# qzs634/Probabilistic-Multiplanar-Unet

Hardware: AMD Instinct MI355X
Metric: 2D slices/sec fwd+bwd, 256×256×1 batch32 U-Net; Dice vs ref (higher is better)
Workload: dtype fp32; 1 GPU; c2: UNet(n_channels=1, n_classes=1, num_filters=[64, 128, 256, 512, 1024]), 256x256x1 slices, fwd+BCE+bwd+clip(0.1)+SGD(0.9) per step, fp32; global_batch=32, per_gpu_batch=32, parallelism=dp1

## Files before the change

### probabilistic-multiplanar-unet_amd/csrc/conv3x3_wino4.hip

```cpp
#include <string.h>
#include <stdlib.h>
#include <utility>
#include "pmu_common.h"
#include "pmu_lds.h"

namespace {

constexpr int TX = 8, TY = 8;
constexpr int OW = 4 * TX, OH = 4 * TY;
constexpr int HW = OW + 2, HH = OH + 2;
constexpr int BK = 8;
constexpr int GP = 36;
constexpr int ROWF = 312;
constexpr int ROWU = ROWF / 4;
constexpr int A_FLOATS = HH * ROWF;
constexpr int CO = 32;
constexpr int NC = 36;
constexpr int U_FLOATS = BK * CO * NC;
constexpr int STAGE = A_FLOATS + U_FLOATS;
constexpr int NT = 512;
constexpr int A_UNITS = A_FLOATS / 4;
constexpr int NGL = (A_UNITS + NT - 1) / NT;
constexpr int UGL = (U_FLOATS / 4 + NT - 1) / NT;
constexpr int RED_FLOATS = 8 * 16 * 2;
static_assert(U_FLOATS % (4 * 256) == 0, "U of whole wave DMA instructions");
static_assert((2 * STAGE + RED_FLOATS) * 4 <= 160 * 1024, "LDS");

struct W4Args {
  const float* x;
  const float* wp;
  const float* bias;
  float* out0;
  float* out1;
  float* part;
  int H, W, KC, NOUT, split, bw, bh, nco, cpb;
  int prio;
  int ts, tc;
  int N;
  const float* bz;
  const float* bcoef;
  const float* bmean;
  const float* binv;
};

constexpr int upos(int ch, int cl) { return cl < 16 ? 16 * ch + cl : 32 + 2 * ch + (cl - 16); }

__device__ __forceinline__ void g6(const double (&g)[3], double (&t)[6]) {
  t[0] = g[0] / 4.0;
  t[1] = -(g[0] + g[1] + g[2]) / 6.0;
  t[2] = -(g[0] - g[1] + g[2]) / 6.0;
  t[3] = g[0] / 24.0 + g[1] / 12.0 + g[2] / 6.0;
  t[4] = g[0] / 24.0 - g[1] / 12.0 + g[2] / 6.0;
  t[5] = g[2];
}

__device__ __forceinline__ void pack_wino4_body(const float* __restrict__ w, int Cout, int Cin, int dgrad,
                                                float* __restrict__ wp, int bid) {
  constexpr int SEG = BK * CO * NC;
  __shared__ float4 seg4[SEG / 4];
  const int NOUT = dgrad ? Cin : Cout, KC = dgrad ? Cout : Cin;
  const int nch = (KC + BK - 1) / BK;
  const int ch = bid % nch, jb = bid / nch;
  for (int f = threadIdx.x; f < BK * CO; f += blockDim.x) {
    const int col = dgrad ? f % CO : f / BK, kl = dgrad ? f / CO : f % BK;
    const int j = jb * CO + col, k = ch * BK + kl;
    double g[3][3];
    for (int a = 0; a < 3; ++a)
      for (int b = 0; b < 3; ++b) {
        double v = 0.0;
        if (j < NOUT && k < KC)
          v = dgrad ? w[((long long)k * Cin + j) * 9 + (2 - a) * 3 + (2 - b)] : w[((long long)j * Cin + k) * 9 + a * 3 + b];
        g[a][b] = v;
      }
    double t[6][3];
    for (int b = 0; b < 3; ++b) {
      const double col3[3] = {g[0][b], g[1][b], g[2][b]};
      double o[6];
      g6(col3, o);
      for (int a = 0; a < 6; ++a) t[a][b] = o[a];
    }
    float u[36];
    for (int a = 0; a < 6; ++a) {
      const double row3[3] = {t[a][0], t[a][1], t[a][2]};
      double o[6];
      g6(row3, o);
      for (int b = 0; b < 6; ++b) u[6 * a + b] = (float)o[b];
    }
    float row[36];
    for (int c = 0; c < 36; ++c) row[upos(c / 18, c % 18)] = u[c];
    float4* d = seg4 + (kl * CO + col) * (NC / 4);
    for (int q = 0; q < 9; ++q) d[q] = make_float4(row[4 * q], row[4 * q + 1], row[4 * q + 2], row[4 * q + 3]);
  }
  __syncthreads();
  float4* dst = reinterpret_cast<float4*>(wp + (long long)bid * SEG);
  for (int i = threadIdx.x; i < SEG / 4; i += blockDim.x) dst[i] = seg4[i];
}
__global__ __launch_bounds__(256) void pack_wino4_kernel(const float* __restrict__ w, int Cout, int Cin, int dgrad,
                                                         float* __restrict__ wp) {
  pack_wino4_body(w, Cout, Cin, dgrad, wp, blockIdx.x);
}
__global__ __launch_bounds__(256) void pack_wino4_multi_kernel(const pmu_pack_job* __restrict__ jobs, int njobs,
                                                               int dgrad) {
  const pmu_pack_job& j = jobs[pmu_job_of(jobs, njobs, blockIdx.x)];
  pack_wino4_body(j.w, j.Cout, j.Cin, dgrad, (float*)j.dst, blockIdx.x - j.block0);
}

__device__ __forceinline__ void bt6(float d0, float d1, float d2, float d3, float d4, float d5, float& r0, float& r1,
                                    float& r2, float& r3, float& r4, float& r5) {
  r0 = fmaf(-5.f, d2, fmaf(4.f, d0, d4));
  const float a = fmaf(-4.f, d2, d4), b = fmaf(-4.f, d1, d3);
  r1 = a + b;
  r2 = a - b;
  const float c = d4 - d2, e = d3 - d1;
  r3 = fmaf(2.f, e, c);
  r4 = fmaf(-2.f, e, c);
  r5 = fmaf(-5.f, d3, fmaf(4.f, d1, d5));
}

__device__ __forceinline__ void input_transform4(const float (&d)[36], float (&v)[36]) {
  float t[36];
#pragma unroll
  for (int j = 0; j < 6; ++j)
    bt6(d[j], d[6 + j], d[12 + j], d[18 + j], d[24 + j], d[30 + j], t[j], t[6 + j], t[12 + j], t[18 + j], t[24 + j],
        t[30 + j]);
#pragma unroll
  for (int a = 0; a < 6; ++a)
    bt6(t[6 * a], t[6 * a + 1], t[6 * a + 2], t[6 * a + 3], t[6 * a + 4], t[6 * a + 5], v[6 * a], v[6 * a + 1],
        v[6 * a + 2], v[6 * a + 3], v[6 * a + 4], v[6 * a + 5]);
}

__device__ __forceinline__ void at4(float m0, float m1, float m2, float m3, float m4, float m5, float& y0, float& y1,
                                    float& y2, float& y3) {
  const float s12 = m1 + m2, d12 = m1 - m2, s34 = m3 + m4, d34 = m3 - m4;
  y0 = m0 + s12 + s34;
  y1 = fmaf(2.f, d34, d12);
  y2 = fmaf(4.f, s34, s12);
  y3 = fmaf(8.f, d34, d12) + m5;
}

template <int E>
struct PatchOff {
  static constexpr int value = ((E / 6) * ROWF + ((E % 6) >> 2) * GP + ((E % 6) & 3) * 8) * 4;
};
template <int E0, int N>
__device__ __forceinline__ void load_patch_part(unsigned pa, float (&d)[36]) {
  if constexpr (N > 0) {
    d[E0] = lds_b32<PatchOff<E0>::value>(pa);
    load_patch_part<E0 + 1, N - 1>(pa, d);
  }
}

template <int CH>
__device__ __forceinline__ void input_transform_half(const float (&d)[36], float (&v)[18]) {
  float t[18];
#pragma unroll
  for (int j = 0; j < 6; ++j) {
    const float d0 = d[j], d1 = d[6 + j], d2 = d[12 + j], d3 = d[18 + j], d4 = d[24 + j], d5 = d[30 + j];
    if (CH == 0) {
      t[j] = fmaf(-5.f, d2, fmaf(4.f, d0, d4));
      const float a = fmaf(-4.f, d2, d4), b = fmaf(-4.f, d1, d3);
      t[6 + j] = a + b;
      t[12 + j] = a - b;
    } else {
      const float c = d4 - d2, e = d3 - d1;
      t[j] = fmaf(2.f, e, c);
      t[6 + j] = fmaf(-2.f, e, c);
      t[12 + j] = fmaf(-5.f, d3, fmaf(4.f, d1, d5));
    }
  }
#pragma unroll
  for (int a = 0; a < 3; ++a)
    bt6(t[6 * a], t[6 * a + 1], t[6 * a + 2], t[6 * a + 3], t[6 * a + 4], t[6 * a + 5], v[6 * a], v[6 * a + 1],
        v[6 * a + 2], v[6 * a + 3], v[6 * a + 4], v[6 * a + 5]);
}

template <int CH, int G>
__device__ __forceinline__ void w4_uread(unsigned ua, float4 (&ur)[3][2], float2 (&ut)[2]) {
  if constexpr (G < 4) {
    ur[G % 3][0] = lds_b128<upos(CH, 4 * G) * 4>(ua);
    ur[G % 3][1] = lds_b128<(16 * NC + upos(CH, 4 * G)) * 4>(ua);
  } else {
    ut[0] = lds_b64<upos(CH, 16) * 4>(ua);
    ut[1] = lds_b64<(16 * NC + upos(CH, 16)) * 4>(ua);
  }
}

template <int CH, int G, bool PF>
__device__ __forceinline__ void w4_group(unsigned ua, const float (&v)[18], float4 (&ur)[3][2], float2 (&ut)[2],
                                         f32x4 (&acc)[2][18], unsigned pn, float (&dn)[36]) {
  if constexpr (G > 0) wait_lgkm<(PF && G == 4) ? 12 : 2 * ((G + 2 < 4 ? G + 2 : 4) - G)>();
  __builtin_amdgcn_sched_barrier(0);
  if constexpr (G < 4) {
    constexpr int c0 = 4 * G;
#pragma unroll
    for (int h = 0; h < 2; ++h) {
      const float4 q = ur[G % 3][h];
      acc[h][c0 + 0] = mfma16(v[c0 + 0], q.x, acc[h][c0 + 0]);
      acc[h][c0 + 1] = mfma16(v[c0 + 1], q.y, acc[h][c0 + 1]);
      acc[h][c0 + 2] = mfma16(v[c0 + 2], q.z, acc[h][c0 + 2]);
      acc[h][c0 + 3] = mfma16(v[c0 + 3], q.w, acc[h][c0 + 3]);
    }
  } else {
#pragma unroll
    for (int h = 0; h < 2; ++h) {
      acc[h][16] = mfma16(v[16], ut[h].x, acc[h][16]);
      acc[h][17] = mfma16(v[17], ut[h].y, acc[h][17]);
    }
  }
  __builtin_amdgcn_sched_barrier(0);
  if constexpr (G + 3 <= 4) w4_uread<CH, G + 3>(ua, ur, ut);
  if constexpr (PF && G == 3) load_patch_part<0, 12>(pn, dn);
  if constexpr (PF && G == 4) load_patch_part<12, 24>(pn, dn);
}

template <int CH, bool PF>
__device__ __forceinline__ void w4_chunk(unsigned pa, unsigned ua, f32x4 (&acc)[2][18]) {
  float d[36], v[18];
  float4 ur[3][2];
  float2 ut[2];
  load_patch_part<0, 36>(pa, d);
  w4_uread<CH, 0>(ua, ur, ut);
  w4_uread<CH, 1>(ua, ur, ut);
  w4_uread<CH, 2>(ua, ur, ut);
  wait_lgkm<4>();
  __builtin_amdgcn_sched_barrier(0);
  input_transform_half<CH>(d, v);
  __builtin_amdgcn_sched_barrier(0);
  const unsigned pa1 = pa + 4, ua1 = ua + CO * NC * 4;
  w4_group<CH, 0, PF>(ua, v, ur, ut, acc, pa1, d);
  w4_group<CH, 1, PF>(ua, v, ur, ut, acc, pa1, d);
  w4_group<CH, 2, PF>(ua, v, ur, ut, acc, pa1, d);
  w4_group<CH, 3, PF>(ua, v, ur, ut, acc, pa1, d);
  w4_group<CH, 4, PF>(ua, v, ur, ut, acc, pa1, d);
  if constexpr (!PF) load_patch_part<0, 36>(pa1, d);
  w4_uread<CH, 0>(ua1, ur, ut);
  w4_uread<CH, 1>(ua1, ur, ut);
  w4_uread<CH, 2>(ua1, ur, ut);
  wait_lgkm<4>();
  __builtin_amdgcn_sched_barrier(0);
  input_transform_half<CH>(d, v);
  __builtin_amdgcn_sched_barrier(0);
  w4_group<CH, 0, false>(ua1, v, ur, ut, acc, pa1, d);
  w4_group<CH, 1, false>(ua1, v, ur, ut, acc, pa1, d);
  w4_group<CH, 2, false>(ua1, v, ur, ut, acc, pa1, d);
  w4_group<CH, 3, false>(ua1, v, ur, ut, acc, pa1, d);
  w4_group<CH, 4, false>(ua1, v, ur, ut, acc, pa1, d);
}

template <int CH>
__device__ __forceinline__ void w4_col_half(float d0, float d1, float d2, float d3, float d4, float d5, float& r0,
                                            float& r1, float& r2) {
  if (CH == 0) {
    r0 = fmaf(-5.f, d2, fmaf(4.f, d0, d4));
    const float a = fmaf(-4.f, d2, d4), b = fmaf(-4.f, d1, d3);
    r1 = a + b;
    r2 = a - b;
  } else {
    const float c = d4 - d2, e = d3 - d1;
    r0 = fmaf(2.f, e, c);
    r1 = fmaf(-2.f, e, c);
    r2 = fmaf(-5.f, d3, fmaf(4.f, d1, d5));
  }
}
template <int CH, int J>
__device__ __forceinline__ void w4_col_read(unsigned pa, float2 (&c)[5]) {
  c[0] = lds_b64<PatchOff<6 * CH + J>::value>(pa);
  c[1] = lds_b64<PatchOff<6 * CH + 6 + J>::value>(pa);
  c[2] = lds_b64<PatchOff<6 * CH + 12 + J>::value>(pa);
  c[3] = lds_b64<PatchOff<6 * CH + 18 + J>::value>(pa);
  c[4] = lds_b64<PatchOff<6 * CH + 24 + J>::value>(pa);
}
template <int CH, int J>
__device__ __forceinline__ void w4_col_tf(const float2 (&c)[5], float (&t0)[18], float (&t1)[18]) {
  if (CH == 0) {
    w4_col_half<0>(c[0].x, c[1].x, c[2].x, c[3].x, c[4].x, 0.f, t0[J], t0[6 + J], t0[12 + J]);
    w4_col_half<0>(c[0].y, c[1].y, c[2].y, c[3].y, c[4].y, 0.f, t1[J], t1[6 + J], t1[12 + J]);
  } else {
    w4_col_half<1>(0.f, c[0].x, c[1].x, c[2].x, c[3].x, c[4].x, t0[J], t0[6 + J], t0[12 + J]);
    w4_col_half<1>(0.f, c[0].y, c[1].y, c[2].y, c[3].y, c[4].y, t1[J], t1[6 + J], t1[12 + J]);
  }
}
template <int CH>
__device__ __forceinline__ void w4_row_pass(const float (&t)[18], float (&v)[18]) {
#pragma unroll
  for (int a = 0; a < 3; ++a)
    bt6(t[6 * a], t[6 * a + 1], t[6 * a + 2], t[6 * a + 3], t[6 * a + 4], t[6 * a + 5], v[6 * a], v[6 * a + 1],
        v[6 * a + 2], v[6 * a + 3], v[6 * a + 4], v[6 * a + 5]);
}

template <int CH>
__device__ __forceinline__ void w4_chunk64(unsigned pa, unsigned ua, f32x4 (&acc)[2][18]) {
  float t0[18], t1[18], v[18];
  float2 cA[5], cB[5];
  float4 ur[3][2];
  float2 ut[2];
  w4_col_read<CH, 0>(pa, cA);
  w4_col_read<CH, 1>(pa, cB);
  wait_lgkm<5>();
  __builtin_amdgcn_sched_barrier(0);
  w4_col_tf<CH, 0>(cA, t0, t1);
  __builtin_amdgcn_sched_barrier(0);
  w4_col_read<CH, 2>(pa, cA);
  wait_lgkm<5>();
  __builtin_amdgcn_sched_barrier(0);
  w4_col_tf<CH, 1>(cB, t0, t1);
  __builtin_amdgcn_sched_barrier(0);
  w4_col_read<CH, 3>(pa, cB);
  wait_lgkm<5>();
  __builtin_amdgcn_sched_barrier(0);
  w4_col_tf<CH, 2>(cA, t0, t1);
  __builtin_amdgcn_sched_barrier(0);
  w4_col_read<CH, 4>(pa, cA);
  wait_lgkm<5>();
  __builtin_amdgcn_sched_barrier(0);
  w4_col_tf<CH, 3>(cB, t0, t1);
  __builtin_amdgcn_sched_barrier(0);
  w4_col_read<CH, 5>(pa, cB);
  w4_uread<CH, 0>(ua, ur, ut);
  w4_uread<CH, 1>(ua, ur, ut);
  w4_uread<CH, 2>(ua, ur, ut);
  wait_lgkm<11>();
  __builtin_amdgcn_sched_barrier(0);
  w4_col_tf<CH, 4>(cA, t0, t1);
  __builtin_amdgcn_sched_barrier(0);
  wait_lgkm<6>();
  __builtin_amdgcn_sched_barrier(0);
  w4_col_tf<CH, 5>(cB, t0, t1);
  w4_row_pass<CH>(t0, v);
  __builtin_amdgcn_sched_barrier(0);
  wait_lgkm<4>();
  __builtin_amdgcn_sched_barrier(0);
  float dn[36];
  w4_group<CH, 0, false>(ua, v, ur, ut, acc, 0u, dn);
  w4_group<CH, 1, false>(ua, v, ur, ut, acc, 0u, dn);
  w4_group<CH, 2, false>(ua, v, ur, ut, acc, 0u, dn);
  w4_group<CH, 3, false>(ua, v, ur, ut, acc, 0u, dn);
  w4_group<CH, 4, false>(ua, v, ur, ut, acc, 0u, dn);
  const unsigned ua1 = ua + CO * NC * 4;
  w4_uread<CH, 0>(ua1, ur, ut);
  w4_uread<CH, 1>(ua1, ur, ut);
  w4_uread<CH, 2>(ua1, ur, ut);
  w4_row_pass<CH>(t1, v);
  wait_lgkm<4>();
  __builtin_amdgcn_sched_barrier(0);
  w4_group<CH, 0, false>(ua1, v, ur, ut, acc, 0u, dn);
  w4_group<CH, 1, false>(ua1, v, ur, ut, acc, 0u, dn);
  w4_group<CH, 2, false>(ua1, v, ur, ut, acc, 0u, dn);
  w4_group<CH, 3, false>(ua1, v, ur, ut, acc, 0u, dn);
  w4_group<CH, 4, false>(ua1, v, ur, ut, acc, 0u, dn);
}

template <int CH>
__device__ __forceinline__ void w4_partial(const f32x4 (&acc)[2][18], int h, int r, float (&P)[16]) {
  float R[3][4];
#pragma unroll
  for (int a = 0; a < 3; ++a)
    at4(acc[h][6 * a][r], acc[h][6 * a + 1][r], acc[h][6 * a + 2][r], acc[h][6 * a + 3][r], acc[h][6 * a + 4][r],
        acc[h][6 * a + 5][r], R[a][0], R[a][1], R[a][2], R[a][3]);
#pragma unroll
  for (int q = 0; q < 4; ++q) {
    if (CH == 0) {
      const float s = R[1][q] + R[2][q], df = R[1][q] - R[2][q];
      P[q] = R[0][q] + s;
      P[4 + q] = df;
      P[8 + q] = s;
      P[12 + q] = df;
    } else {
      const float s = R[0][q] + R[1][q], df = R[0][q] - R[1][q];
      P[q] = s;
      P[4 + q] = 2.f * df;
      P[8 + q] = 4.f * s;
      P[12 + q] = fmaf(8.f, df, R[2][q]);
    }
  }
}

template <bool DGRAD, bool BNR, int CH>
__device__ __forceinline__ void wino4_epilogue(const W4Args& a, int n, int h0, int w0, int j0, int spatial,
                                               const f32x4 (&acc)[2][18], float* xb, float* red, float bias) {
  const int tid = threadIdx.x, lane = tid & 63, wave = tid >> 6, kk = lane >> 4;
  const int tg = wave & 3, partner = tg + 4 * (1 - CH);
  const int j = j0 + 16 * CH + (lane & 15);
  const bool jok = j < a.NOUT;
  float* dst;
  int ld;
  if (!DGRAD) { dst = a.out0 + j; ld = a.NOUT; }
  else if (j < a.split) { dst = a.out0 + j; ld = a.split; }
  else { dst = a.out1 + (j - a.split); ld = a.NOUT - a.split; }
  float s1 = 0.f, s2 = 0.f;
  float bsc = 0.f, bsh = 0.f, bmu = 0.f, bis = 0.f;
  if (BNR && jok) {
    bsc = a.bcoef[j];
    bsh = a.bcoef[a.NOUT + j];
    bmu = a.bmean[j];
    bis = a.binv[j];
  }
#pragma unroll
  for (int rho = 0; rho < 2; ++rho) {
    if (rho) __syncthreads();
#pragma unroll
    for (int rr = 0; rr < 2; ++rr) {
      float P[16];
      w4_partial<CH>(acc, 1 - CH, 2 * rho + rr, P);
#pragma unroll
      for (int e = 0; e < 16; ++e) xb[((wave * 2 + rr) * 16 + e) * 64 + lane] = P[e];
    }
    __syncthreads();
#pragma unroll
    for (int rr = 0; rr < 2; ++rr) {
      const int r = 2 * rho + rr;
      const int t = 4 * kk + r;
      const int oh = h0 + 4 * (2 * tg + (t >> 3)), ow = w0 + 4 * (t & 7);
      float zt[16];
      if (BNR) {
        const int jc = min(j, a.NOUT - 1);
#pragma unroll
        for (int e = 0; e < 16; ++e) {
          const int hh2 = oh + (e >> 2), ww = ow + (e & 3);
          const long long pix = ((long long)n * a.H + min(hh2, a.H - 1)) * a.W + min(ww, a.W - 1);
          zt[e] = a.bz[pix * a.NOUT + jc];
        }
      }
      float P[16];
      w4_partial<CH>(acc, CH, r, P);
      float xv[16];
#pragma unroll
      for (int e = 0; e < 16; ++e) xv[e] = xb[((partner * 2 + rr) * 16 + e) * 64 + lane];
#pragma unroll
      for (int e = 0; e < 16; ++e) asm volatile("" : "+v"(xv[e]));
#pragma unroll
      for (int p = 0; p < 4; ++p) {
        const int hh2 = oh + p;
        float* rowp = dst + (long long)((long long)n * a.H + min(hh2, a.H - 1)) * a.W * ld;
#pragma unroll
        for (int q = 0; q < 4; ++q) {
          const int ww = ow + q;
          const float v = P[4 * p + q] + xv[4 * p + q] + bias;
          const bool ok = jok && hh2 < a.H && ww < a.W;
          if (!DGRAD) {
            const float m = ok ? v : 0.f;
            s1 += m;
            s2 = fmaf(m, m, s2);
          } else if (BNR) {
            const float zz = zt[4 * p + q];
            const float g = (ok && fmaf(zz, bsc, bsh) > 0.f) ? v : 0.f;
            s1 += g;
            s2 = fmaf(g, (zz - bmu) * bis, s2);
          }
          if (!ok) continue;
          PMU_DCHECK((((long long)n * a.H + hh2) * a.W + ww) < (long long)a.N * a.H * a.W && j < a.NOUT, PMU_DBG_OUTPUT);
          rowp[(unsigned)(ww * ld)] = v;
        }
      }
    }
  }
  if (a.part) {
    s1 += __shfl_xor(s1, 16, 64);
    s2 += __shfl_xor(s2, 16, 64);
    s1 += __shfl_xor(s1, 32, 64);
    s2 += __shfl_xor(s2, 32, 64);
    if (lane < 16) {
      red[(wave * 16 + lane) * 2 + 0] = s1;
      red[(wave * 16 + lane) * 2 + 1] = s2;
    }
    __syncthreads();
    if (tid < CO) {
      const int jj = j0 + tid, hf = tid >> 4, l = tid & 15;
      if (jj < a.NOUT) {
        float t1 = 0.f, t2 = 0.f;
#pragma unroll
        for (int g = 0; g < 4; ++g) {
          t1 += red[((4 * hf + g) * 16 + l) * 2 + 0];
          t2 += red[((4 * hf + g) * 16 + l) * 2 + 1];
        }
        PMU_DCHECK(spatial < (long long)a.N * a.bh * a.bw, PMU_DBG_WORKSPACE);
        a.part[((long long)spatial * 2 + 0) * a.NOUT + jj] = t1;
        a.part[((long long)spatial * 2 + 1) * a.NOUT + jj] = t2;
      }
    }
  }
  __syncthreads();
}

struct W4Block {
  int n, h0, w0, cob0, spatial, nchunks, npass;
  unsigned gin;
  unsigned gzero;
};

template <bool DGRAD, bool BNR, int CH, int PM>
__device__ __forceinline__ void wino4_main(const W4Args& a, const W4Block& B, const unsigned (&goff)[NGL],
                                           float* smem) {
  float* red = smem + 2 * STAGE;
  const int tid = threadIdx.x, lane = tid & 63, wave = tid >> 6;
  const int nchunks = B.nchunks, total = B.npass * nchunks;
  const float* wsrc = a.wp + (long long)B.cob0 * nchunks * U_FLOATS;
  const unsigned uoff = 16u * tid;
  const int wave_off = wave * 256;
  const unsigned gin = B.gin;
#define PMU_FETCH4(GI, BUF)                                                                                 \
  {                                                                                                        \
    const int p_ = (GI) / nchunks;                                                                         \
    const int c_ = (GI) - p_ * nchunks;                                                                    \
    const int cs_ = ((B.cob0 + p_) & 1) ? nchunks - 1 - c_ : c_;                                           \
    const int k0_ = cs_ * BK;                                                                              \
    PMU_DCHECK(k0_ + BK <= a.KC, PMU_DBG_OPERAND);                                                         \
    float* b_ = (BUF);                                                                                     \
    const char* xb_ = reinterpret_cast<const char*>(a.x + k0_);                                            \
    _Pragma("unroll") for (int r = 0; r < NGL; ++r)                                                        \
      if ((gin >> r) & 1u) PMU_GLDS(xb_ + goff[r], b_ + 4 * (r * NT) + wave_off)                           \
    const char* s_ = reinterpret_cast<const char*>(wsrc + ((long long)p_ * nchunks + cs_) * U_FLOATS) + uoff; \
    float* d_ = b_ + A_FLOATS + wave_off;                                                                  \
    _Pragma("unroll") for (int r = 0; r < UGL; ++r)                                                        \
      if (r * NT * 4 + (wave + 1) * 256 <= U_FLOATS) PMU_GLDS(s_ + 16 * NT * r, d_ + 4 * NT * r)          \
  }
  const int t = lane & 15, kk = lane >> 4, tg = wave & 3;
  const int pbase = 4 * (2 * tg + (t >> 3)) * ROWF + GP * (t & 7) + 2 * kk;
  const int ubase = A_FLOATS + (2 * kk * CO + t) * NC;
  f32x4 acc[2][18];
#pragma unroll
  for (int h = 0; h < 2; ++h)
#pragma unroll
    for (int c = 0; c < 18; ++c) acc[h][c] = f32x4{0.f, 0.f, 0.f, 0.f};

  PMU_FETCH4(0, smem)
  asm volatile("s_waitcnt vmcnt(0)" ::: "memory");
  __syncthreads();
  for (int p = 0; p < B.npass; ++p) {
    const int j0 = (B.cob0 + p) * CO;
    const int jb = j0 + 16 * CH + t;
    const float bias = (!DGRAD && a.bias && jb < a.NOUT) ? a.bias[jb] : 0.f;
    int gi = p * nchunks;
    for (int ch = 0; ch < nchunks; ++ch, ++gi) {
      float* cur = smem + (gi & 1) * STAGE;
      if (gi + 1 < total) PMU_FETCH4(gi + 1, smem + ((gi + 1) & 1) * STAGE)
      const unsigned pa = lds_addr(cur + pbase), ua = lds_addr(cur + ubase);
      if constexpr (PM == 2) w4_chunk64<CH>(pa, ua, acc);
      else w4_chunk<CH, PM == 1>(pa, ua, acc);
      asm volatile("s_waitcnt vmcnt(0)" ::: "memory");
      __syncthreads();
    }
    int ne = B.n, h0e = B.h0, w0e = B.w0;
    asm volatile("" : "+s"(ne), "+s"(h0e), "+s"(w0e));
    float* xb = smem + ((gi - 1) & 1) * STAGE;
    wino4_epilogue<DGRAD, BNR, CH>(a, ne, h0e, w0e, j0, B.spatial, acc, xb, red, bias);
    if (p + 1 < B.npass) {
#pragma unroll
      for (int r = 0; r < NGL; ++r)
        if ((B.gzero >> r) & 1u) *reinterpret_cast<float4*>(xb + 4 * (r * NT + tid)) = make_float4(0.f, 0.f, 0.f, 0.f);
      __syncthreads();
    }
#pragma unroll
    for (int h = 0; h < 2; ++h)
#pragma unroll
      for (int c = 0; c < 18; ++c) acc[h][c] = f32x4{0.f, 0.f, 0.f, 0.f};
  }
#undef PMU_FETCH4
}

template <bool DGRAD, bool BNR, int PM>
__global__ __launch_bounds__(NT, 1) void conv3x3_wino4_kernel(W4Args a) {
  __shared__ __attribute__((aligned(16))) float smem[2 * STAGE + RED_FLOATS];
  const int tid = threadIdx.x;
  const int lb = pmu_xcd_block(blockIdx.x, gridDim.x);
  const int ncog = (a.nco + a.cpb - 1) / a.cpb;
  W4Block B;
  int cg, sp;
  if (a.tc > 0) {
    const int gsz = a.ts * a.tc, g = lb / gsz, i = lb - g * gsz;
    const int gpr = ncog / a.tc;
    cg = (g % gpr) * a.tc + i % a.tc;
    sp = (g / gpr) * a.ts + i / a.tc;
  } else {
    cg = lb % ncog;
    sp = lb / ncog;
  }
  B.cob0 = cg * a.cpb;
  B.spatial = sp;
  const int bx = sp % a.bw; sp /= a.bw;
  const int by = sp % a.bh;
  B.n = sp / a.bh;
  B.h0 = by * OH;
  B.w0 = bx * OW;
  const int KC = a.KC;
  B.nchunks = KC / BK;
  B.npass = a.cpb < a.nco - B.cob0 ? a.cpb : a.nco - B.cob0;
  PMU_DCHECK(B.n < a.N && B.cob0 < a.nco, PMU_DBG_GRID);

  unsigned goff[NGL];
  unsigned gin = 0u, gzero = 0u;
#pragma unroll
  for (int r = 0; r < NGL; ++r) {
    const int u = r * NT + tid;
    const int hr = u / ROWU, wu = u - hr * ROWU;
    const int g = wu / 9, w9 = wu - 9 * g;
    const int px = 4 * g + (w9 >> 1);
    const bool data = u < A_UNITS && w9 < 8 && px < HW;
    const int h = B.h0 - 1 + hr, w = B.w0 - 1 + px;
    const bool in = data && h >= 0 && w >= 0 && h < a.H && w < a.W;
    goff[r] = in ? (unsigned)(((((long long)B.n * a.H + h) * a.W + w) * KC + 4 * (w9 & 1)) * 4) : 0u;
    PMU_DCHECK(!in || (((long long)B.n * a.H + h) * a.W + w) < (long long)a.N * a.H * a.W, PMU_DBG_OPERAND);
    gin |= in ? (1u << r) : 0u;
    gzero |= (data && !in) ? (1u << r) : 0u;
    if (data && !in) {
      *reinterpret_cast<float4*>(smem + 4 * u) = make_float4(0.f, 0.f, 0.f, 0.f);
      *reinterpret_cast<float4*>(smem + STAGE + 4 * u) = make_float4(0.f, 0.f, 0.f, 0.f);
    }
  }
  B.gin = gin;
  B.gzero = gzero;
  if (a.prio && (tid >> 8)) __builtin_amdgcn_s_setprio(1);
  if (tid >> 8) wino4_main<DGRAD, BNR, 1, PM>(a, B, goff, smem);
  else wino4_main<DGRAD, BNR, 0, PM>(a, B, goff, smem);
}

int launch_wino4(const float* x, int KC, int N, int H, int W, const float* wp, const float* bias, int NOUT,
                 float* out0, float* out1, int split, float* part, bool dgrad, void* stream,
                 const float* bz = nullptr, const float* bcoef = nullptr, const float* bmean = nullptr,
                 const float* binv = nullptr) {
  const pmu_wino_call c{x, KC, N, H, W, wp, bias, NOUT, out0, out1, split, part, bz, bcoef, bmean, binv};
  return pmu_wino_launch<W4Args>(c, OW, OH, BK, CO, "PMU_WINO4_CPB", "PMU_WINO4_MINWG",
                                 [&](W4Args& a, long long spatial, dim3 grid) {
    static const int pf = pmu_variant_int("PMU_WINO4_PF", 0);
    static const int b32 = pmu_variant_int("PMU_WINO4_B32", 0);
    const int pm = pf ? 1 : b32 ? 0 : 2;
    static const int prio = pmu_variant_int("PMU_WINO4_PRIO", 0);
    a.prio = prio;
    static const int grp = pmu_variant_int("PMU_WINO4_GROUP", 1);
    if (grp) {
      const int ncog = pmu_cdiv(a.nco, a.cpb);
      const int tc = ncog < 8 ? ncog : 8, ts = 32 / tc;
      if (ncog % tc == 0 && spatial % ts == 0 && tc > 1 && ts > 1) { a.tc = tc; a.ts = ts; }
    }
    hipStream_t st = (hipStream_t)stream;
#ifdef PMU_EXPERIMENTS
    if (dgrad && bz && pm == 0) hipLaunchKernelGGL((conv3x3_wino4_kernel<true, true, 0>), grid, dim3(NT), 0, st, a);
    else if (dgrad && bz) hipLaunchKernelGGL((conv3x3_wino4_kernel<true, true, 2>), grid, dim3(NT), 0, st, a);
    else if (dgrad && pm == 1) hipLaunchKernelGGL((conv3x3_wino4_kernel<true, false, 1>), grid, dim3(NT), 0, st, a);
    else if (dgrad && pm == 0) hipLaunchKernelGGL((conv3x3_wino4_kernel<true, false, 0>), grid, dim3(NT), 0, st, a);
    else if (dgrad) hipLaunchKernelGGL((conv3x3_wino4_kernel<true, false, 2>), grid, dim3(NT), 0, st, a);
    else if (pm == 1) hipLaunchKernelGGL((conv3x3_wino4_kernel<false, false, 1>), grid, dim3(NT), 0, st, a);
    else if (pm == 0) hipLaunchKernelGGL((conv3x3_wino4_kernel<false, false, 0>), grid, dim3(NT), 0, st, a);
    else hipLaunchKernelGGL((conv3x3_wino4_kernel<false, false, 2>), grid, dim3(NT), 0, st, a);
#else
    (void)pm;
    if (dgrad && bz) hipLaunchKernelGGL((conv3x3_wino4_kernel<true, true, 2>), grid, dim3(NT), 0, st, a);
    else if (dgrad) hipLaunchKernelGGL((conv3x3_wino4_kernel<true, false, 2>), grid, dim3(NT), 0, st, a);
    else return (int)PMU_ERR_ARG;
#endif
    PMU_CHECK_LAUNCH();
    return (int)PMU_OK;
  });
}

}

extern "C" int pmu_conv3x3_tiles_wino4(int N, int H, int W) { return N * pmu_cdiv(H, OH) * pmu_cdiv(W, OW); }

extern "C" size_t pmu_conv3x3_packed_size_wino4(int Cout, int Cin, int dgrad) {
  const int NOUT = dgrad ? Cin : Cout, KC = dgrad ? Cout : Cin;
  return (size_t)pmu_cdiv(NOUT, CO) * pmu_cdiv(KC, BK) * U_FLOATS * sizeof(float);
}

extern "C" int pmu_conv3x3_pack_wino4(const float* w, int Cout, int Cin, int dgrad, float* wp, void* stream) {
  PMU_REQUIRE(w && wp && Cout > 0 && Cin > 0);
  const int NOUT = dgrad ? Cin : Cout, KC = dgrad ? Cout : Cin;
  const unsigned segs = (unsigned)(pmu_cdiv(NOUT, CO) * pmu_cdiv(KC, BK));
  hipLaunchKernelGGL(pack_wino4_kernel, dim3(segs), dim3(256), 0, (hipStream_t)stream, w, Cout, Cin, dgrad, wp);
  PMU_CHECK_LAUNCH();
  return PMU_OK;
}

#ifdef PMU_EXPERIMENTS
extern "C" int pmu_conv3x3_fwd_wino4(const float* xt, int Cin, int N, int H, int W, const float* wp, const float* bias,
                                     int Cout, float* z, float* part, void* stream) {
  return launch_wino4(xt, Cin, N, H, W, wp, bias, Cout, z, nullptr, Cout, part, false, stream);
}
#endif

extern "C" int pmu_conv3x3_dgrad_wino4(const float* dzt, int Cout, int N, int H, int W, const float* wp, int Cin,
                                       int Csplit, float* dx0, float* dx1, void* stream) {
  PMU_REQUIRE(Csplit > 0 && Csplit <= Cin && (Csplit == Cin || dx1));
  return launch_wino4(dzt, Cout, N, H, W, wp, nullptr, Cin, dx0, dx1, Csplit, nullptr, true, stream);
}

extern "C" int pmu_conv3x3_dgrad_wino4_bnr(const float* dzt, int Cout, int N, int H, int W, const float* wp, int Cin,
                                           float* dx, const float* z, const float* coef, const float* mean,
                                           const float* invstd, float* part, void* stream) {
  PMU_REQUIRE(z && coef && mean && invstd && part);
  return launch_wino4(dzt, Cout, N, H, W, wp, nullptr, Cin, dx, nullptr, Cin, part, true, stream, z, coef, mean,
                      invstd);
}

extern "C" int pmu_conv3x3_pack_wino4_blocks(int Cout, int Cin, int dgrad) {
  const int NOUT = dgrad ? Cin : Cout, KC = dgrad ? Cout : Cin;
  return pmu_cdiv(NOUT, CO) * pmu_cdiv(KC, BK);
}

extern "C" int pmu_conv3x3_pack_wino4_multi(const pmu_pack_job* jobs, int njobs, int blocks, int dgrad, void* stream) {
  PMU_REQUIRE(jobs && njobs > 0 && blocks > 0);
  hipLaunchKernelGGL(pack_wino4_multi_kernel, dim3((unsigned)blocks), dim3(256), 0, (hipStream_t)stream, jobs, njobs,
                     dgrad);
  PMU_CHECK_LAUNCH();
  return PMU_OK;
}
```

Measured before the change: 717.2 slices/s.

## Stagger Winograd-4 dgrad operand fetches across wave halves with split barriers

Splits the 64-channel chunk compute into two stages and splits the double-buffered fetch into separate activation and weight-tile loads. Under the new STAG template, one half of the block issues activation loads and the other half issues weight loads at different points around a mid-chunk barrier, so global-to-LDS traffic overlaps more evenly with compute. It also skips the BN partial-stat reduction for plain dgrad and adds asm register pins. The stagger is on by default for dgrad on large maps, at the cost of an extra barrier per chunk and more intricate buffer-reuse ordering that could race.

```diff
diff --git a/probabilistic-multiplanar-unet_amd/csrc/conv3x3_wino4.hip b/probabilistic-multiplanar-unet_amd/csrc/conv3x3_wino4.hip
--- a/probabilistic-multiplanar-unet_amd/csrc/conv3x3_wino4.hip
+++ b/probabilistic-multiplanar-unet_amd/csrc/conv3x3_wino4.hip
@@ -289,8 +289,8 @@
 }
 
 template <int CH>
-__device__ __forceinline__ void w4_chunk64(unsigned pa, unsigned ua, f32x4 (&acc)[2][18]) {
-  float t0[18], t1[18], v[18];
+__device__ __forceinline__ void w4_chunk64_s0(unsigned pa, unsigned ua, f32x4 (&acc)[2][18], float (&t1)[18]) {
+  float t0[18], v[18];
   float2 cA[5], cB[5];
   float4 ur[3][2];
   float2 ut[2];
@@ -336,7 +336,13 @@
   w4_group<CH, 2, false>(ua, v, ur, ut, acc, 0u, dn);
   w4_group<CH, 3, false>(ua, v, ur, ut, acc, 0u, dn);
   w4_group<CH, 4, false>(ua, v, ur, ut, acc, 0u, dn);
-  const unsigned ua1 = ua + CO * NC * 4;
+}
+template <int CH>
+__device__ __forceinline__ void w4_chunk64_s1(unsigned ua1, f32x4 (&acc)[2][18], const float (&t1)[18]) {
+  float v[18];
+  float4 ur[3][2];
+  float2 ut[2];
+  float dn[36];
   w4_uread<CH, 0>(ua1, ur, ut);
   w4_uread<CH, 1>(ua1, ur, ut);
   w4_uread<CH, 2>(ua1, ur, ut);
@@ -378,7 +384,9 @@
 template <bool DGRAD, bool BNR, int CH>
 __device__ __forceinline__ void wino4_epilogue(const W4Args& a, int n, int h0, int w0, int j0, int spatial,
                                                const f32x4 (&acc)[2][18], float* xb, float* red, float bias) {
-  const int tid = threadIdx.x, lane = tid & 63, wave = tid >> 6, kk = lane >> 4;
+  int tid = threadIdx.x;
+  asm volatile("" : "+v"(tid));
+  const int lane = tid & 63, wave = tid >> 6, kk = lane >> 4;
   const int tg = wave & 3, partner = tg + 4 * (1 - CH);
   const int j = j0 + 16 * CH + (lane & 15);
   const bool jok = j < a.NOUT;
@@ -454,7 +462,7 @@
       }
     }
   }
-  if (a.part) {
+  if ((!DGRAD || BNR) && a.part) {
     s1 += __shfl_xor(s1, 16, 64);
     s2 += __shfl_xor(s2, 16, 64);
     s1 += __shfl_xor(s1, 32, 64);
@@ -482,37 +490,51 @@
   __syncthreads();
 }
 
+__device__ __forceinline__ void w4_barrier() { asm volatile("s_waitcnt lgkmcnt(0)\n\ts_barrier" ::: "memory"); }
+
 struct W4Block {
   int n, h0, w0, cob0, spatial, nchunks, npass;
   unsigned gin;
   unsigned gzero;
 };
 
-template <bool DGRAD, bool BNR, int CH, int PM>
+template <bool DGRAD, bool BNR, int CH, int PM, bool STAG>
 __device__ __forceinline__ void wino4_main(const W4Args& a, const W4Block& B, const unsigned (&goff)[NGL],
                                            float* smem) {
   float* red = smem + 2 * STAGE;
   const int tid = threadIdx.x, lane = tid & 63, wave = tid >> 6;
-  const int nchunks = B.nchunks, total = B.npass * nchunks;
+  const int nchunks = B.nchunks;
   const float* wsrc = a.wp + (long long)B.cob0 * nchunks * U_FLOATS;
   const unsigned uoff = 16u * tid;
   const int wave_off = wave * 256;
   const unsigned gin = B.gin;
-#define PMU_FETCH4(GI, BUF)                                                                                 \
+#define PMU_FETCH4A(P, C, BUF)                                                                              \
   {                                                                                                        \
-    const int p_ = (GI) / nchunks;                                                                         \
-    const int c_ = (GI) - p_ * nchunks;                                                                    \
-    const int cs_ = ((B.cob0 + p_) & 1) ? nchunks - 1 - c_ : c_;                                           \
+    const int cs_ = ((B.cob0 + (P)) & 1) ? nchunks - 1 - (C) : (C);                                        \
     const int k0_ = cs_ * BK;                                                                              \
     PMU_DCHECK(k0_ + BK <= a.KC, PMU_DBG_OPERAND);                                                         \
     float* b_ = (BUF);                                                                                     \
     const char* xb_ = reinterpret_cast<const char*>(a.x + k0_);                                            \
+    unsigned g_ = gin;     \
+    asm volatile("" : "+v"(g_));                                                                           \
     _Pragma("unroll") for (int r = 0; r < NGL; ++r)                                                        \
-      if ((gin >> r) & 1u) PMU_GLDS(xb_ + goff[r], b_ + 4 * (r * NT) + wave_off)                           \
-    const char* s_ = reinterpret_cast<const char*>(wsrc + ((long long)p_ * nchunks + cs_) * U_FLOATS) + uoff; \
-    float* d_ = b_ + A_FLOATS + wave_off;                                                                  \
+      if ((g_ >> r) & 1u) {                                                                                \
+         \
+         \
+        unsigned o_ = goff[r];                                                                             \
+        asm volatile("" : "+v"(o_));                                                                       \
+        PMU_GLDS(xb_ + o_, b_ + 4 * (r * NT) + wave_off)                                                   \
+      }                                                                                                    \
+  }
+#define PMU_FETCH4U(P, C, BUF)                                                                              \
+  {                                                                                                        \
+    const int cs_ = ((B.cob0 + (P)) & 1) ? nchunks - 1 - (C) : (C);                                        \
+    unsigned u_ = uoff;                                                                                    \
+    asm volatile("" : "+v"(u_));                                             \
+    const char* s_ = reinterpret_cast<const char*>(wsrc + ((long long)(P) * nchunks + cs_) * U_FLOATS);    \
+    float* d_ = (BUF) + A_FLOATS + wave_off;                                                               \
     _Pragma("unroll") for (int r = 0; r < UGL; ++r)                                                        \
-      if (r * NT * 4 + (wave + 1) * 256 <= U_FLOATS) PMU_GLDS(s_ + 16 * NT * r, d_ + 4 * NT * r)          \
+      if (r * NT * 4 + (wave + 1) * 256 <= U_FLOATS) PMU_GLDS((s_ + 16 * NT * r) + u_, d_ + 4 * NT * r)   \
   }
   const int t = lane & 15, kk = lane >> 4, tg = wave & 3;
   const int pbase = 4 * (2 * tg + (t >> 3)) * ROWF + GP * (t & 7) + 2 * kk;
@@ -523,7 +545,11 @@
 #pragma unroll
     for (int c = 0; c < 18; ++c) acc[h][c] = f32x4{0.f, 0.f, 0.f, 0.f};
 
-  PMU_FETCH4(0, smem)
+  constexpr bool stag = STAG;
+  static_assert(!STAG || PM == 2, "the stagger splits the b64 chunk");
+
+  PMU_FETCH4A(0, 0, smem)
+  PMU_FETCH4U(0, 0, smem)
   asm volatile("s_waitcnt vmcnt(0)" ::: "memory");
   __syncthreads();
   for (int p = 0; p < B.npass; ++p) {
@@ -531,23 +557,50 @@
     const int jb = j0 + 16 * CH + t;
     const float bias = (!DGRAD && a.bias && jb < a.NOUT) ? a.bias[jb] : 0.f;
     int gi = p * nchunks;
+    if (CH == 1 && stag) {
+      const int c1 = min(nchunks - 1, 1);
+      if (c1 > 0 || p + 1 < B.npass) PMU_FETCH4A(p + 1 - c1, c1, smem + ((gi + 1) & 1) * STAGE)
+      w4_barrier();
+    }
     for (int ch = 0; ch < nchunks; ++ch, ++gi) {
       float* cur = smem + (gi & 1) * STAGE;
-      if (gi + 1 < total) PMU_FETCH4(gi + 1, smem + ((gi + 1) & 1) * STAGE)
+      float* nxt = smem + ((gi + 1) & 1) * STAGE;
+      const bool more = ch + 1 < nchunks || p + 1 < B.npass;
+      const int pn = ch + 1 < nchunks ? p : p + 1, cn = ch + 1 < nchunks ? ch + 1 : 0;
+      if (more && (CH == 0 || !stag)) PMU_FETCH4A(pn, cn, nxt)
+      if (more && (CH == 1 || !stag)) PMU_FETCH4U(pn, cn, nxt)
       const unsigned pa = lds_addr(cur + pbase), ua = lds_addr(cur + ubase);
-      if constexpr (PM == 2) w4_chunk64<CH>(pa, ua, acc);
-      else w4_chunk<CH, PM == 1>(pa, ua, acc);
-      asm volatile("s_waitcnt vmcnt(0)" ::: "memory");
-      __syncthreads();
-    }
+      if constexpr (PM == 2) {
+        float t1[18];
+        w4_chunk64_s0<CH>(pa, ua, acc, t1);
+        if (stag) {
+          if (CH == 1) asm volatile("s_waitcnt vmcnt(0)" ::: "memory");
+          w4_barrier();
+          if (CH == 0) {
+            if (more) PMU_FETCH4U(pn, cn, nxt)
+          } else if (ch + 2 < nchunks || (ch + 1 < nchunks && p + 1 < B.npass)) {
+            PMU_FETCH4A(ch + 2 < nchunks ? p : p + 1, ch + 2 < nchunks ? ch + 2 : 0, cur)
+          }
+        }
+        w4_chunk64_s1<CH>(ua + CO * NC * 4, acc, t1);
+      } else {
+        w4_chunk<CH, PM == 1>(pa, ua, acc);
+      }
+      if (CH == 0 || !stag) asm volatile("s_waitcnt vmcnt(0)" ::: "memory");
+      if (stag) w4_barrier();
+      else __syncthreads();
+    }
+    if (CH == 0 && stag) w4_barrier();
     int ne = B.n, h0e = B.h0, w0e = B.w0;
     asm volatile("" : "+s"(ne), "+s"(h0e), "+s"(w0e));
     float* xb = smem + ((gi - 1) & 1) * STAGE;
     wino4_epilogue<DGRAD, BNR, CH>(a, ne, h0e, w0e, j0, B.spatial, acc, xb, red, bias);
     if (p + 1 < B.npass) {
+      float zr = 0.f;
+      asm volatile("" : "+v"(zr));
 #pragma unroll
       for (int r = 0; r < NGL; ++r)
-        if ((B.gzero >> r) & 1u) *reinterpret_cast<float4*>(xb + 4 * (r * NT + tid)) = make_float4(0.f, 0.f, 0.f, 0.f);
+        if ((B.gzero >> r) & 1u) *reinterpret_cast<float4*>(xb + 4 * (r * NT + tid)) = make_float4(zr, zr, zr, zr);
       __syncthreads();
     }
 #pragma unroll
@@ -555,10 +608,11 @@
 #pragma unroll
       for (int c = 0; c < 18; ++c) acc[h][c] = f32x4{0.f, 0.f, 0.f, 0.f};
   }
-#undef PMU_FETCH4
-}
-
-template <bool DGRAD, bool BNR, int PM>
+#undef PMU_FETCH4A
+#undef PMU_FETCH4U
+}
+
+template <bool DGRAD, bool BNR, int PM, bool STAG = false>
 __global__ __launch_bounds__(NT, 1) void conv3x3_wino4_kernel(W4Args a) {
   __shared__ __attribute__((aligned(16))) float smem[2 * STAGE + RED_FLOATS];
   const int tid = threadIdx.x;
@@ -610,8 +664,8 @@
   B.gin = gin;
   B.gzero = gzero;
   if (a.prio && (tid >> 8)) __builtin_amdgcn_s_setprio(1);
-  if (tid >> 8) wino4_main<DGRAD, BNR, 1, PM>(a, B, goff, smem);
-  else wino4_main<DGRAD, BNR, 0, PM>(a, B, goff, smem);
+  if (tid >> 8) wino4_main<DGRAD, BNR, 1, PM, STAG>(a, B, goff, smem);
+  else wino4_main<DGRAD, BNR, 0, PM, STAG>(a, B, goff, smem);
 }
 
 int launch_wino4(const float* x, int KC, int N, int H, int W, const float* wp, const float* bias, int NOUT,
@@ -626,6 +680,8 @@
     const int pm = pf ? 1 : b32 ? 0 : 2;
     static const int prio = pmu_variant_int("PMU_WINO4_PRIO", 0);
     a.prio = prio;
+    static const int stag_env = pmu_variant_int("PMU_WINO4_STAGGER", 1);
+    const bool stagger = pm == 2 && (stag_env == 2 || (stag_env == 1 && (a.H >= OH || a.W >= OW)));
     static const int grp = pmu_variant_int("PMU_WINO4_GROUP", 1);
     if (grp) {
       const int ncog = pmu_cdiv(a.nco, a.cpb);
@@ -633,18 +689,20 @@
       if (ncog % tc == 0 && spatial % ts == 0 && tc > 1 && ts > 1) { a.tc = tc; a.ts = ts; }
     }
     hipStream_t st = (hipStream_t)stream;
+    if (dgrad && bz && stagger) hipLaunchKernelGGL((conv3x3_wino4_kernel<true, true, 2, true>), grid, dim3(NT), 0, st, a);
+    else if (dgrad && stagger) hipLaunchKernelGGL((conv3x3_wino4_kernel<true, false, 2, true>), grid, dim3(NT), 0, st, a);
 #ifdef PMU_EXPERIMENTS
-    if (dgrad && bz && pm == 0) hipLaunchKernelGGL((conv3x3_wino4_kernel<true, true, 0>), grid, dim3(NT), 0, st, a);
+    else if (dgrad && bz && pm == 0) hipLaunchKernelGGL((conv3x3_wino4_kernel<true, true, 0>), grid, dim3(NT), 0, st, a);
     else if (dgrad && bz) hipLaunchKernelGGL((conv3x3_wino4_kernel<true, true, 2>), grid, dim3(NT), 0, st, a);
     else if (dgrad && pm == 1) hipLaunchKernelGGL((conv3x3_wino4_kernel<true, false, 1>), grid, dim3(NT), 0, st, a);
     else if (dgrad && pm == 0) hipLaunchKernelGGL((conv3x3_wino4_kernel<true, false, 0>), grid, dim3(NT), 0, st, a);
     else if (dgrad) hipLaunchKernelGGL((conv3x3_wino4_kernel<true, false, 2>), grid, dim3(NT), 0, st, a);
+    else if (stagger) hipLaunchKernelGGL((conv3x3_wino4_kernel<false, false, 2, true>), grid, dim3(NT), 0, st, a);
     else if (pm == 1) hipLaunchKernelGGL((conv3x3_wino4_kernel<false, false, 1>), grid, dim3(NT), 0, st, a);
     else if (pm == 0) hipLaunchKernelGGL((conv3x3_wino4_kernel<false, false, 0>), grid, dim3(NT), 0, st, a);
     else hipLaunchKernelGGL((conv3x3_wino4_kernel<false, false, 2>), grid, dim3(NT), 0, st, a);
 #else
-    (void)pm;
-    if (dgrad && bz) hipLaunchKernelGGL((conv3x3_wino4_kernel<true, true, 2>), grid, dim3(NT), 0, st, a);
+    else if (dgrad && bz) hipLaunchKernelGGL((conv3x3_wino4_kernel<true, true, 2>), grid, dim3(NT), 0, st, a);
     else if (dgrad) hipLaunchKernelGGL((conv3x3_wino4_kernel<true, false, 2>), grid, dim3(NT), 0, st, a);
     else return (int)PMU_ERR_ARG;
 #endif
```

Result: no change. 722.3 slices/s, median of 6 (+0.7%).
